# uma-pi1/kge

Hardware: AMD Instinct MI355X
Metric: scored triples/sec (1vsAll, ComplEx d=512) (higher is better)
Workload: dtype bf16; 1 GPU; FB15k-237 shape ComplEx d=512 1vsAll scoring, bf16 tables, f32 scores: the score_sp and score_po blocks of a batch per step (KgeModel.score_sp_po), batches issued in groups of `group` -- one persistent launch per group (kge_score_queries_multi), which also builds the next group's query vectors; group k on HIP stream k % `group_launches_in_flight`; score rows on a 256-byte pitch; num_entities_per_gpu=14541, num_relations=237, dim=512, batch=512, group=8, group_launches_in_flight=1, parallelism=single GPU, queries=split (q_hi + q_lo)

## Files before the change

### kge_amd/csrc/score_pairs_bf16_v8.hip

```cpp
#include "common.hpp"
#include "bf16_queries.hpp"
#include <atomic>
#include <cstdlib>

namespace kge {

constexpr int V8_UT = 32;
constexpr int V8_BAND_CAP = 255;
constexpr int V8_PB = 14;
constexpr unsigned int V8_DROP = 0x80000000u;

struct V8Args {
  Operand TG;
  long long n, m;
  int rgn1;
  int sides;
  int chunks;
  int nbatch;
  long long q_stride;
  long long out_stride;
  long long out2_off, ldo;
  int nunits, su, wpx;
  float* out;
  const u32x4* qf;
  unsigned long long* dbg;
  NextQ nx;
};

#define KGE_V8_DMA(D, VO, P) \
  KGE_STALL(__LINE__ + 7000); \
  asm volatile("s_mov_b32 m0, %0\n\ts_nop 0\n\tglobal_load_lds_dwordx4 %1, %2" : : "s"(D), "v"(VO), "s"(P) : "memory", "m0")

template <int SCORER, int SPLIT, int AUX, int VAR = 0>
__global__ __launch_bounds__(512, 1) void pairs_bf16_v8_kernel(V8Args a) {
  constexpr int HH = 256;
  constexpr int NKB = 2 * HH / 16;
  constexpr int ROWB = 4 * HH;
  constexpr int UNITB = V8_UT * ROWB;
  constexpr int NBUF = 4;
  constexpr int SMEM = NBUF * UNITB;
  constexpr int RW = SPLIT ? 16 : 32;
  constexpr int NST = SPLIT ? 8 : 16;
  constexpr int PF = SPLIT ? 4 : 8;
  static_assert(NKB % PF == 0 && PF <= 8, "look-ahead depth");
  constexpr int FR0 = 12;
  constexpr int VMN_STEADY = (NST > 15 ? 1 : 0) + NST + 4 + V8_PB / 2;
  constexpr int VMN = VMN_STEADY - 2;
  static_assert(VMN <= (NST > 15 ? 9 : 1) + (NKB - FR0 - 14) + 4 + V8_PB / 2, "the chain behind the cold chain");
  __shared__ __attribute__((aligned(16))) unsigned char smem[SMEM];
  if (a.n < 0) smem[threadIdx.x] = 0;

  const int b = blockIdx.x;
  const int x = b & 7, j = b >> 3;
  const int tid = threadIdx.x, lane = tid & 63;
  const int wave = __builtin_amdgcn_readfirstlane(tid >> 6);
  int u_lo = x * a.su;
  int sux = a.nunits - u_lo;
  if (sux > a.su) sux = a.su;
  const int P = a.nbatch * a.sides * a.chunks;
  const int g0 = 0;
  int g1 = 0, pair0 = 0, pstep = a.wpx;
  if (sux > 0) {
    if (P >= a.wpx) {
      pair0 = j;
      g1 = j < P ? ((P - j + a.wpx - 1) / a.wpx) * sux : 0;
    } else {
      const int nsub = a.wpx / P;
      if (j < P * nsub) {
        pair0 = j % P;
        const int sub = j / P;
        const int lo = (int)((long long)sux * sub / nsub), hi = (int)((long long)sux * (sub + 1) / nsub);
        u_lo += lo;
        sux = hi - lo;
        g1 = sux;
      }
    }
  }

  int dbg_i = 0;
  auto stamp = [&]() {
    if (a.dbg != nullptr && tid == 0 && dbg_i < 32) a.dbg[(long long)blockIdx.x * 64 + dbg_i] = __builtin_readcyclecounter();
    ++dbg_i;
  };
  auto stamp_at = [&](int slot) {
    if (a.dbg != nullptr && tid == 0) a.dbg[(long long)blockIdx.x * 64 + slot] = __builtin_readcyclecounter();
  };

  if (g1 > g0) {
    stamp();
    const unsigned char* const tgb = (const unsigned char*)a.TG.base;
    const long long tld2 = a.TG.ld * 2;
    const long long m = a.m;
    const unsigned int lane16 = (unsigned int)lane << 4;
    const int r4 = 4 * wave;
    const unsigned int dx0 = (unsigned int)((r4 & 15) << 4);
    int dq = g0;
    int du = g0 % sux;
    const int ulast = (g1 - 1) % sux;
    auto dma_piece = [&](int un, int ks, auto kc) __attribute__((always_inline)) {
      constexpr int kk = decltype(kc)::value;
      long long r = (long long)(u_lo + un) * V8_UT + r4 + kk;
      if (r >= m) r = m - 1;
      const unsigned char* pk = tgb + r * tld2;
      const unsigned int dk = (unsigned int)((ks & (NBUF - 1)) * UNITB + (r4 + kk) * ROWB);
      const unsigned int vo = lane16 ^ (dx0 + (unsigned int)(kk << 4));
      KGE_V8_DMA(dk, vo, pk);
    };
    auto dma_advance = [&]() __attribute__((always_inline)) {
      ++dq;
      if (++du == sux) du = 0;
    };
    auto fill_unit = [&](int k) __attribute__((always_inline)) {
      const int un = dq < g1 ? du : ulast;
      v4_static_for<0, 4>([&](auto kc) __attribute__((always_inline)) { dma_piece(un, k, kc); });
      dma_advance();
    };

    const int fi = lane & 31, fh = lane >> 5;
    bf16x8 afr[NKB];
    unsigned int bp[8];
#pragma unroll
    for (int t = 0; t < 8; ++t) bp[t] = (unsigned int)(fi * ROWB + (((2 * t + fh) ^ (fi & 15)) << 4));
    bf16x8 bq[PF];
    auto bread = [&](bf16x8& dst, auto kc) __attribute__((always_inline)) {
      constexpr int kb = decltype(kc)::value;
      const unsigned int addr = bp[kb & 7];
      asm volatile("ds_read_b128 %0, %1 offset:%2" : "=v"(dst) : "v"(addr), "i"((kb >> 3) * 256) : "memory");
    };
    const unsigned int ldo4 = (unsigned int)(a.ldo * 4);
    const unsigned int svo = (unsigned int)(((long long)(4 * fh) * a.ldo + fi) * 4);
    __amdgpu_buffer_rsrc_t srs = __builtin_amdgcn_make_buffer_rsrc((void*)a.out, 0, 0, 0x00020000);
    auto store_q = [&](const f32x16& acc, auto qc, unsigned int vo, unsigned int colb) __attribute__((always_inline)) {
      constexpr int q = decltype(qc)::value;
      constexpr int r = SPLIT ? (q & 3) + 8 * (q >> 2) : q;
      constexpr int rowc = SPLIT ? 8 * (r >> 3) + (r & 3) : 8 * (r >> 2) + (r & 3);
      const unsigned int vr = vo + (unsigned int)rowc * ldo4;
      float v = acc[r];
      if constexpr (SPLIT) {
        const float lo = acc[r + 4];
        v = v + lo;
      }
      if constexpr (VAR & 1) {
        asm volatile("" : : "v"(v), "v"(vr));
      } else {
        __builtin_amdgcn_raw_buffer_store_b32(__builtin_bit_cast(unsigned int, v), srs, vr, colb, AUX);
      }
    };
    auto unit_vo = [&](int cu, unsigned int& colb) __attribute__((always_inline)) -> unsigned int {
      const long long col0 = (long long)(u_lo + cu) * V8_UT;
      colb = (unsigned int)(col0 * 4);
      return (col0 + V8_UT <= m || col0 + fi < m) ? svo : V8_DROP;
    };

    f32x16 acc0, acc1;
    auto chain = [&](int ks, f32x16& acc, const f32x16& prev, unsigned int vo, unsigned int colb, auto cold, auto&& frag)
        __attribute__((always_inline)) {
      constexpr bool COLD = decltype(cold)::value;
      const unsigned int bdelta = ((ks + 1) & (NBUF - 1)) ? (unsigned int)UNITB : (unsigned int)(-(NBUF - 1) * UNITB);
      int un = dq < g1 ? du : ulast;
      v4_static_for<0, NKB>([&](auto kc) __attribute__((always_inline)) {
        constexpr int kb = decltype(kc)::value;
        asm volatile("s_waitcnt lgkmcnt(%0)" ::"i"(PF - 1) : "memory");
        if constexpr (kb == V8_PB) {
          asm volatile("s_waitcnt vmcnt(%0)" ::"i"(COLD ? 25 : VMN) : "memory");
          KGE_BARRIER();
        }
        __builtin_amdgcn_sched_barrier(0);
        if constexpr (kb == 0) {
          const f32x16 zero = {0, 0, 0, 0, 0, 0, 0, 0, 0, 0, 0, 0, 0, 0, 0, 0};
          acc = __builtin_amdgcn_mfma_f32_32x32x16_bf16(afr[0], bq[0], zero, 0, 0, 0);
        } else {
          acc = __builtin_amdgcn_mfma_f32_32x32x16_bf16(afr[kb], bq[kb % PF], acc, 0, 0, 0);
        }
        if constexpr (kb + PF == NKB) {
#pragma unroll
          for (int t = 0; t < 8; ++t) asm volatile("v_add_u32 %0, %1, %0" : "+v"(bp[t]) : "s"(bdelta));
        }
        bread(bq[kb % PF], std::integral_constant<int, (kb + PF) % NKB>{});
        if constexpr ((kb & 1) == 0 && kb / 2 < NST) store_q(prev, std::integral_constant<int, kb / 2>{}, vo, colb);
        if constexpr (COLD && kb < NKB - FR0) frag(std::integral_constant<int, FR0 + kb>{});
        if constexpr (COLD && kb < 14 && (kb & 3) == 1) dma_piece(un, ks + 2, std::integral_constant<int, kb / 4>{});
        if constexpr (COLD && kb == 14) {
          dma_advance();
          un = dq < g1 ? du : ulast;
        }
        if constexpr (kb >= 17 && ((kb - 17) & 3) == 0) dma_piece(un, ks + 3, std::integral_constant<int, (kb - 17) / 4>{});
      });
      dma_advance();
      stamp();
    };
    using Cold = std::true_type;
    using Warm = std::false_type;
    auto nofrag = [](auto) {};

    int g = g0, ks = 0;
    int pair = pair0;
    const int cu = 0;
    bool first = true;
    while (g < g1) {
      const int cnt = sux;
      const int per = a.sides * a.chunks;
      const int lb = pair / per, rem = pair - lb * per;
      const int side = rem / a.chunks, ch = rem - side * a.chunks;
      const long long rb = (long long)ch * (8 * RW) + RW * wave;
      long long rows_here = rb < a.n ? (a.n - rb < RW ? a.n - rb : RW) : 0;
      float* const ob = a.out + (long long)lb * a.out_stride + (side ? a.out2_off : 0) + (rows_here > 0 ? rb : 0) * a.ldo;
      srs = __builtin_amdgcn_make_buffer_rsrc((void*)ob, 0, (int)(rows_here * a.ldo * 4), 0x00020000);
      int grp = 2 * ch + (wave >> 2);
      if (grp >= a.rgn1) grp = a.rgn1 - 1;
      grp += side * a.rgn1;
      const unsigned char* const gbase = (const unsigned char*)(a.qf + (long long)lb * a.q_stride + (long long)grp * 4 * NKB * 64);
      unsigned int flo;
      const unsigned char* fb;
      int frange;
      if constexpr (SPLIT) {
        const int part = (fi >> 3) & 1, rr = 16 * (wave & 3) + 8 * (fi >> 4) + (fi & 7);
        flo = (unsigned int)((((2 * part + (rr >> 5)) * NKB) * 64 + (rr & 31) + 32 * fh) * 16);
        fb = gbase;
        frange = 4 * NKB * 1024;
      } else {
        flo = (unsigned int)(lane * 16);
        fb = gbase + (wave & 3) * (NKB * 1024);
        frange = NKB * 1024;
      }
      const __amdgpu_buffer_rsrc_t frs = __builtin_amdgcn_make_buffer_rsrc((void*)fb, 0, frange, 0x00020000);
      auto load_fragments = [&](auto lo, auto hi) __attribute__((always_inline)) {
        v4_static_for<decltype(lo)::value, decltype(hi)::value>([&](auto kc) __attribute__((always_inline)) {
          constexpr int kb = decltype(kc)::value;
          afr[kb] = __builtin_bit_cast(bf16x8, __builtin_amdgcn_raw_buffer_load_b128(frs, flo + kb * 1024, 0, 16 ));
        });
      };
      using C0 = std::integral_constant<int, 0>;
      using CF = std::integral_constant<int, FR0>;
      using C32 = std::integral_constant<int, NKB>;
      unsigned int pvo = V8_DROP, pcolb = 0;
      if (first) {
        fill_unit(0);
        load_fragments(C0{}, CF{});
        asm volatile("s_waitcnt vmcnt(%0)" ::"i"(FR0) : "memory");
        KGE_BARRIER();
        stamp();
        fill_unit(1);
        v4_static_for<0, PF>([&](auto jc) __attribute__((always_inline)) { bread(bq[decltype(jc)::value], jc); });
        first = false;
        chain(ks, acc0, acc1, pvo, pcolb, Cold{}, [&](auto kc) __attribute__((always_inline)) {
          load_fragments(kc, std::integral_constant<int, decltype(kc)::value + 1>{});
        });
      } else {
        load_fragments(C0{}, C32{});
        chain(ks, acc0, acc1, pvo, pcolb, Warm{}, nofrag);
      }
      pvo = unit_vo(cu, pcolb);
      ++ks;
      int i = 1;
      for (; i + 1 < cnt; i += 2) {
        chain(ks, acc1, acc0, pvo, pcolb, Warm{}, nofrag);
        pvo = unit_vo(cu + i, pcolb);
        chain(ks + 1, acc0, acc1, pvo, pcolb, Warm{}, nofrag);
        pvo = unit_vo(cu + i + 1, pcolb);
        ks += 2;
      }
      if (i < cnt) {
        chain(ks, acc1, acc0, pvo, pcolb, Warm{}, nofrag);
        pvo = unit_vo(cu + i, pcolb);
        ++ks;
        v4_static_for<0, NST>([&](auto qc) __attribute__((always_inline)) { store_q(acc1, qc, pvo, pcolb); });
      } else {
        v4_static_for<0, NST>([&](auto qc) __attribute__((always_inline)) { store_q(acc0, qc, pvo, pcolb); });
      }
      g += cnt;
      pair += pstep;
    }
    asm volatile("s_waitcnt lgkmcnt(0)" ::: "memory");
    if constexpr (PF == 8)
      asm volatile("" : : "v"(bq[0]), "v"(bq[1]), "v"(bq[2]), "v"(bq[3]), "v"(bq[4]), "v"(bq[5]), "v"(bq[6]), "v"(bq[7]));
    else
      asm volatile("" : : "v"(bq[0]), "v"(bq[1]), "v"(bq[2]), "v"(bq[3]));
    stamp_at(34);
  }
  if (a.nx.qf != nullptr)
    v4_build_queries<SCORER, HH, SPLIT>(a.nx, (long long)blockIdx.x * 512 + threadIdx.x, (long long)gridDim.x * 512);
}

void v6_set_stamps(unsigned long long* p);
unsigned long long* v6_get_stamps();

int run_pairs_bf16_v8_store256(const Operand& TG, bool split, bool two_sided, long long n, long long m, int nbatch,
                               const void* qf, long long q_stride_bytes, float* out, long long out_stride, long long ldo,
                               long long out2_off, int sc1, int reserve_cus, hipStream_t st);

static int v8_cu_count() {
  static std::atomic<int> cache[64];
  int dev = 0;
  if (hipGetDevice(&dev) != hipSuccess) return 0;
  if (dev >= 0 && dev < 64) {
    const int c = cache[dev].load(std::memory_order_relaxed);
    if (c > 0) return c;
  }
  int v = 0;
  if (hipDeviceGetAttribute(&v, hipDeviceAttributeMultiprocessorCount, dev) != hipSuccess) return 0;
  if (dev >= 0 && dev < 64) cache[dev].store(v, std::memory_order_relaxed);
  return v;
}

static int g_v8_launches[2] = {0, 0};
int v8_launch_count(int which) { return (which == 0 || which == 1) ? __atomic_load_n(&g_v8_launches[which], __ATOMIC_RELAXED) : -1; }

template <int SCORER, int SPLIT>
static int launch_v8(V8Args& a, int sc1, hipStream_t st) {
  int cus = v8_cu_count();
  (void)cus;
  __atomic_fetch_add(&g_v8_launches[0], 1, __ATOMIC_RELAXED);
  const dim3 grid(8 * a.wpx), block(512);
#ifdef KGE_V8_PROBES
  if constexpr (SCORER == KGE_COMPLEX && SPLIT == 1) {
    if (sw(SW_V8_VAR) == 1) {
      hipLaunchKernelGGL((pairs_bf16_v8_kernel<SCORER, SPLIT, 2, 1>), grid, block, 0, st, a);
      return hipGetLastError() == hipSuccess ? KGE_OK : KGE_ERR_LAUNCH;
    }
  }
#endif
  if (sc1 == 1)
    hipLaunchKernelGGL((pairs_bf16_v8_kernel<SCORER, SPLIT, 16>), grid, block, 0, st, a);
  else if (sc1 == 2)
    hipLaunchKernelGGL((pairs_bf16_v8_kernel<SCORER, SPLIT, 2>), grid, block, 0, st, a);
  else if (sc1 == 3)
    hipLaunchKernelGGL((pairs_bf16_v8_kernel<SCORER, SPLIT, 18>), grid, block, 0, st, a);
  else
    hipLaunchKernelGGL((pairs_bf16_v8_kernel<SCORER, SPLIT, 0>), grid, block, 0, st, a);
  return hipGetLastError() == hipSuccess ? KGE_OK : KGE_ERR_LAUNCH;
}

int run_pairs_bf16_v8(int scorer, bool split, const Operand& TG, bool two_sided, int d, long long n, long long m,
                      int nbatch, const void* qf, long long q_stride_bytes, float* out, long long out_stride,
                      long long ldo, long long out2_off, hipStream_t st, unsigned long long* dbg, const NextQ& nx,
                      int reserve_cus) {
  if ((d != 512 && d != 256) || TG.idx.ptr != nullptr || qf == nullptr || nbatch < 1) return KGE_ERR_UNSUPPORTED;
  const long long e = sw(SW_V8);
  if (e == 0) return KGE_ERR_UNSUPPORTED;
  if (nbatch == 1 && e != 1) return KGE_ERR_UNSUPPORTED;
  if (TG.ld * 2 >= (1LL << 28) || ldo >= (1LL << 24)) return KGE_ERR_UNSUPPORTED;
  if ((q_stride_bytes & 15) || ((uintptr_t)qf & 15)) return KGE_ERR_INVALID_ARG;
  const long long rgr = split ? 64 : 128;
  const long long rgn1 = (n + rgr - 1) / rgr;
  const long long pairs = (long long)nbatch * (two_sided ? 2 : 1) * ((rgn1 + 1) / 2);
  const long long nunits = (m + V8_UT - 1) / V8_UT;
  if (rgn1 > (1 << 20) || pairs * nunits >= (1LL << 30)) return KGE_ERR_UNSUPPORTED;
  int cus = v8_cu_count() - reserve_cus;
  if (cus > 256) cus = 256;
  if (cus < 8) cus = 8;
  V8Args a{};
  a.TG = TG;
  a.n = n;
  a.m = m;
  a.rgn1 = (int)rgn1;
  a.sides = two_sided ? 2 : 1;
  a.chunks = (int)((rgn1 + 1) / 2);
  a.nbatch = nbatch;
  a.q_stride = q_stride_bytes / 16;
  a.out_stride = out_stride;
  a.out2_off = out2_off;
  a.ldo = ldo;
  a.nunits = (int)nunits;
  a.su = (int)((nunits + 7) / 8);
  a.wpx = cus / 8;
  a.out = out;
  a.qf = (const u32x4*)qf;
  a.dbg = dbg != nullptr ? dbg : v6_get_stamps();
  a.nx = nx;
  const long long sc1e = sw(SW_V4_STORE_SC1);
  const bool st_aligned = (ldo & 7) == 0 && (out2_off & 7) == 0 && (out_stride & 7) == 0 && ((uintptr_t)out & 31) == 0;
  const double bytes = (double)nbatch * (double)n * (double)m * 4.0 * (two_sided ? 2 : 1);
  const int sc1 = sc1e >= 0 ? (int)sc1e : (!st_aligned ? 0 : (bytes > 160e6 ? 2 : (bytes <= 48e6 ? 1 : 0)));
  if (d == 256) {
    if (nx.qf != nullptr) return KGE_ERR_INVALID_ARG;
    const int pol = sc1e >= 0 ? (int)(sc1e & 3) : (st_aligned && bytes > 1e9 ? 1 : 0);
    const int rc = run_pairs_bf16_v8_store256(TG, split, two_sided, n, m, nbatch, qf, q_stride_bytes, out, out_stride, ldo,
                                              out2_off, pol, reserve_cus, st);
    if (rc == KGE_OK) __atomic_fetch_add(&g_v8_launches[0], 1, __ATOMIC_RELAXED);
    return rc;
  }
#define KGE_V8L(SC) return split ? launch_v8<SC, 1>(a, sc1, st) : launch_v8<SC, 0>(a, sc1, st)
  if (scorer == KGE_COMPLEX) { KGE_V8L(KGE_COMPLEX); }
  if (scorer == KGE_DISTMULT) { KGE_V8L(KGE_DISTMULT); }
#undef KGE_V8L
  return KGE_ERR_UNSUPPORTED;
}


struct V8RankArgs {
  Operand TG;
  long long n, m;
  int rgn1, sides, chunks;
  int nunits, su, wpx;
  const u32x4* qf;
  unsigned long long* dbg;
  CeArgs ce;
};

template <int SCORER, int HH, int SPLIT, int PROBE = 0, int BAND = 0>
__global__ __launch_bounds__(512, 1) void pairs_bf16_v8_rank_kernel(V8RankArgs a) {
  static_assert(!BAND || !SPLIT, "the band launch runs the q_hi chains only");
  constexpr bool DUP = SPLIT && HH == 256;
  constexpr int PARTS = (SPLIT && HH == 128) ? 2 : 1;
  constexpr int FSETS = PARTS;
  constexpr int NT = (HH == 128 && !SPLIT) ? 2 : 1;
  constexpr int NACC = NT * PARTS;
  constexpr int UT = V8_UT * NT;
  constexpr int NKB = 2 * HH / 16;
  constexpr int ROWB = 4 * HH;
  constexpr int SPR = ROWB / 16;
  constexpr int RPP = 64 / SPR;
  constexpr int UNITB = UT * ROWB;
  constexpr int SUBB = V8_UT * ROWB;
  constexpr int NBUF = 4;
  constexpr int SMEM = NBUF * UNITB;
  constexpr int NP = UNITB / 1024 / 8;
  constexpr int RW = DUP ? 16 : 32;
  constexpr int PF = 4;
  constexpr int PB = NKB == 32 ? 14 : 6;
  constexpr bool RAWFAST = HH == 128;
  __shared__ __attribute__((aligned(16))) unsigned char smem[SMEM];
  if (a.n < 0) smem[threadIdx.x] = 0;

  const int b = blockIdx.x;
  const int x = b & 7, j = b >> 3;
  const int tid = threadIdx.x, lane = tid & 63;
  const int wave = __builtin_amdgcn_readfirstlane(tid >> 6);
  int u_lo = x * a.su;
  int sux = a.nunits - u_lo;
  if (sux > a.su) sux = a.su;
  const int P = a.sides * a.chunks;
  const int g0 = 0;
  int g1 = 0, pair0 = 0, pstep = a.wpx;
  if (sux > 0) {
    if (P >= a.wpx) {
      pair0 = j;
      g1 = j < P ? ((P - j + a.wpx - 1) / a.wpx) * sux : 0;
    } else {
      const int nsub = a.wpx / P;
      if (j < P * nsub) {
        pair0 = j % P;
        const int sub = j / P;
        const int lo = (int)((long long)sux * sub / nsub), hi = (int)((long long)sux * (sub + 1) / nsub);
        u_lo += lo;
        sux = hi - lo;
        g1 = sux;
      }
    }
  }
  if (g1 <= g0) return;
  int dbg_i = 0;
  auto stamp = [&]() {
    if (a.dbg != nullptr && tid == 0 && dbg_i < 32) a.dbg[(long long)blockIdx.x * 64 + dbg_i] = __builtin_readcyclecounter();
    ++dbg_i;
  };
  stamp();
  if (a.dbg != nullptr && tid == 0) a.dbg[(long long)blockIdx.x * 64 + 42] = wall_clock64();

  const unsigned char* const tgb = (const unsigned char*)a.TG.base;
  const long long tld2 = a.TG.ld * 2;
  const long long m = a.m;
  const int lr = lane / SPR, slot = lane % SPR;
  const int rp0 = wave * NP * RPP;
  int dq = g0, du = g0 % sux;
  const int ulast = (g1 - 1) % sux;
  auto dma_piece = [&](int un, int ks, auto kc) __attribute__((always_inline)) {
    constexpr int kk = decltype(kc)::value;
    const int ru = rp0 + kk * RPP;
    const long long r0 = (long long)(u_lo + un) * UT + ru;
    const unsigned int dk = (unsigned int)((ks & (NBUF - 1)) * UNITB + ru * ROWB);
    const unsigned int sw = (unsigned int)((slot ^ ((ru + lr) & 15)) << 4);
    const long long rb = r0 < m ? r0 : m - 1;
    const unsigned char* pk = tgb + rb * tld2;
    unsigned int vo = sw;
    if constexpr (RPP > 1) {
      const int left = (int)(m - 1 - rb < RPP - 1 ? m - 1 - rb : RPP - 1);
      vo += (unsigned int)((lr < left ? lr : left) * (int)tld2);
    }
    KGE_V8_DMA(dk, vo, pk);
  };
  auto dma_advance = [&]() __attribute__((always_inline)) {
    ++dq;
    if (++du == sux) du = 0;
  };
#pragma unroll
  for (int k = 0; k < NBUF - 1; ++k) {
    const int un = dq < g1 ? du : ulast;
    v4_static_for<0, NP>([&](auto kc) __attribute__((always_inline)) { dma_piece(un, k, kc); });
    dma_advance();
  }

  const int fi = lane & 31, fh = lane >> 5;
  bf16x8 afr[FSETS][NKB];
  unsigned int bp[8];
#pragma unroll
  for (int t = 0; t < 8; ++t) bp[t] = (unsigned int)(fi * ROWB + (((2 * t + fh) ^ (fi & 15)) << 4));
  bf16x8 bq[NT][PF];
  auto bread = [&](bf16x8& dst, auto kc, auto ac) __attribute__((always_inline)) {
    constexpr int kb = decltype(kc)::value, sub = decltype(ac)::value;
    const unsigned int addr = bp[kb & 7];
    asm volatile("ds_read_b128 %0, %1 offset:%2" : "=v"(dst) : "v"(addr), "i"((kb >> 3) * 256 + sub * SUBB) : "memory");
  };

  const CeArgs& ce = a.ce;
  const bool counts_here = DUP ? ((fi >> 3) & 1) == 0 : true;
  float rk_t = 0.0f, rk_al = 0.0f;
  float rk_hi = 0.0f, rk_lo = 0.0f;
  int bl_cnt = 0;
  u32x4* bl_list = nullptr;
  bool rk_slow = false, rk_noraw = false;
  int rk_g = 0, rk_c = 0, rk_fg[2] = {0, 0}, rk_fc[2] = {0, 0}, rk_fn[2] = {0, 0};
  const unsigned char* rk_base = (const unsigned char*)a.qf;
  unsigned int rk_off = 0;
  int orow_cur = 0;
  int side_cur = 0;
  auto rk_spread = [](unsigned int d) __attribute__((always_inline)) -> unsigned int {
    return (d & 0xfu) | ((d & 0xf0u) << 4) | ((d & 0xf00u) << 8) | ((d & 0xf000u) << 12);
  };
  auto full_score = [&](float v) __attribute__((always_inline)) -> float {
    if constexpr (DUP) {
      const float o = __builtin_bit_cast(
          float, __builtin_amdgcn_update_dpp(0, __builtin_bit_cast(int, v), 0x128 , 0xf, 0xf, false));
      return v + o;
    } else {
      return v;
    }
  };
  auto rank_unit = [&](const f32x16& pv, int cu, int sub, unsigned int w0, unsigned int w1, bool count_g = true)
      __attribute__((always_inline)) -> unsigned int {
    unsigned int g, c;
    if (BAND && rk_slow) {
      g = 0u;
      c = 0x0f0f0f0fu;
    } else if (rk_slow) {
      g = c = 0u;
#pragma unroll
      for (int r = 0; r < 16; ++r) {
        int g0_ = 0, c0_ = 0;
        count_one(full_score(pv[r]), rk_t, ce.rk_atol, ce.rk_rtol, g0_, c0_);
        const unsigned int bit = 1u << (8 * (r >> 2) + (r & 3));
        g |= g0_ ? bit : 0u;
        c |= c0_ ? bit : 0u;
      }
    } else {
      unsigned int ng = 0u, nc = 0u;
#pragma unroll
      for (int r = 15; r >= 0; --r) {
        float xq;
        asm("v_max_f32 %0, 0xff800000, %1" : "=v"(xq) : "v"(full_score(pv[r])));
        const float e = xq - rk_t;
        ng = __builtin_amdgcn_alignbit(ng, __builtin_bit_cast(unsigned int, rk_al - e), 31);
        nc = __builtin_amdgcn_alignbit(nc, __builtin_bit_cast(unsigned int, rk_al - __builtin_fabsf(e)), 31);
      }
      g = rk_spread(ng & 0xffffu);
      c = rk_spread(~nc & 0xffffu);
    }
    const long long c0t = ((long long)(u_lo + cu) * NT + sub) * V8_UT;
    unsigned int mine = counts_here ? (0x0f0f0f0fu << (4 * fh)) : 0u;
    const long long rem = m - c0t;
    if (rem < V8_UT) mine &= rem > 0 ? (1u << rem) - 1u : 0u;
    g = (g << (4 * fh)) & mine;
    c = (c << (4 * fh)) & mine;
    if (!count_g) return c;
    rk_g += __builtin_popcount(g);
    if constexpr (!BAND) rk_c += __builtin_popcount(c);
    const unsigned int ww[2] = {w0 & mine, w1 & mine};
#pragma unroll
    for (int k = 0; k < 2; ++k) {
      if (k < ce.rk_nfilt) {
        rk_fg[k] += __builtin_popcount(g & ww[k]);
        if constexpr (!BAND) rk_fc[k] += __builtin_popcount(c & ww[k]);
        rk_fn[k] += __builtin_popcount(ww[k]);
      }
    }
    return c;
  };
  auto rank_unit_raw = [&](const f32x16& pv) __attribute__((always_inline)) -> int {
    int g = 0, c2 = 0;
#pragma unroll
    for (int r = 0; r < 16; ++r) {
      const float x = full_score(pv[r]);
      g += x > rk_hi ? 1 : 0;
      c2 += x >= rk_lo ? 1 : 0;
    }
    rk_g += g;
    if constexpr (!BAND) rk_c += c2 - g;
    return c2 - g;
  };
  auto rank_flush = [&]() __attribute__((always_inline)) {
    const int G = rk_g + __shfl_xor(rk_g, 32, 64), C = rk_c + __shfl_xor(rk_c, 32, 64);
    const bool wr = counts_here && orow_cur < a.n && fh == 0;
    unsigned long long* rank = ce.rk_rank[side_cur] + orow_cur;
    unsigned long long* ties = ce.rk_ties[side_cur] + orow_cur;
    if (wr && G != 0) atomicAdd(rank, (unsigned long long)G);
    if (wr && C != 0) atomicAdd(ties, (unsigned long long)C);
    const int fc = rk_t == -__builtin_inff() ? 1 : 0;
#pragma unroll
    for (int k = 0; k < 2; ++k) {
      if (k < ce.rk_nfilt) {
        const int FG = rk_fg[k] + __shfl_xor(rk_fg[k], 32, 64), FC = rk_fc[k] + __shfl_xor(rk_fc[k], 32, 64);
        const int FN = rk_fn[k] + __shfl_xor(rk_fn[k], 32, 64);
        const int Gk = G - FG, Ck = C - FC + fc * FN;
        if (wr && Gk != 0) atomicAdd(rank + (k + 1) * ce.rk_ld, (unsigned long long)Gk);
        if (wr && Ck != 0) atomicAdd(ties + (k + 1) * ce.rk_ld, (unsigned long long)Ck);
      }
      rk_fg[k] = rk_fc[k] = rk_fn[k] = 0;
    }
    rk_g = rk_c = 0;
  };
  auto load_words = [&](int cu, u32x2 (&w)[NT]) __attribute__((always_inline)) {
#pragma unroll
    for (int sub = 0; sub < NT; ++sub) {
      const unsigned char* wb = rk_base + (ce.rk_nfilt > 0 ? ((long long)(u_lo + cu) * NT + sub) * ce.rk_bits_us * 4 : 0);
      asm volatile("global_load_dwordx2 %0, %1, %2" : "=v"(w[sub]) : "v"(rk_off), "s"(wb) : "memory");
    }
  };

  auto run = [&](auto half) __attribute__((always_inline)) {
    constexpr int HALF = decltype(half)::value;
    constexpr int PBH = HALF ? 0 : PB;
    constexpr int NPV = (PROBE & 2) ? 0 : NP, WV = (PROBE & 8) ? 0 : NT;
    constexpr int VMB = (NBUF - 3) * (NPV + WV) + WV;
    static_assert(VMB + NP + NT < 64, "vmcnt is a 6-bit counter");
    constexpr int VMF = NPV;
    f32x16 acc[NACC];
    u32x2 wc[NT] = {}, wn[NT] = {};
    auto chain = [&](int ks, int cu, int cu_next) __attribute__((always_inline)) {
      const unsigned int bdelta = ((ks + 1) & (NBUF - 1)) ? (unsigned int)UNITB : (unsigned int)(-(NBUF - 1) * UNITB);
      const int un = dq < g1 ? du : ulast;
      v4_static_for<0, NKB>([&](auto kc) __attribute__((always_inline)) {
        constexpr int kb = decltype(kc)::value;
        asm volatile("s_waitcnt lgkmcnt(%0)" ::"i"((PF - 1) * NT) : "memory");
// ... 596 lines not shown
```

Before: 528.1 billion scored triples/s.

## Store score rows as 16-byte lines via DPP quad transpose in split path

```diff
diff --git a/kge_amd/csrc/score_pairs_bf16_v8.hip b/kge_amd/csrc/score_pairs_bf16_v8.hip
--- a/kge_amd/csrc/score_pairs_bf16_v8.hip
+++ b/kge_amd/csrc/score_pairs_bf16_v8.hip
@@ -31,7 +31,30 @@
   KGE_STALL(__LINE__ + 7000); \
   asm volatile("s_mov_b32 m0, %0\n\ts_nop 0\n\tglobal_load_lds_dwordx4 %1, %2" : : "s"(D), "v"(VO), "s"(P) : "memory", "m0")
 
-template <int SCORER, int SPLIT, int AUX, int VAR = 0>
+constexpr int V8_PIECES = 4;
+constexpr int V8_PIECE_SLOT0 = 17, V8_PIECE_STEP = 4;
+constexpr int V8_GROUP_STEPS = 6;
+constexpr int v8_group_slot(int split, int g) { return split ? 6 * g : (g < 2 ? 6 * g : 15 + 7 * (g - 2)); }
+constexpr int v8_stores(int split, int wide) { return wide ? (split ? 2 : 4) : (split ? 8 : 16); }
+constexpr int v8_store_slot(int split, int wide, int q) { return wide ? v8_group_slot(split, q) + V8_GROUP_STEPS - 1 : 2 * q; }
+constexpr int v8_stores_in(int split, int wide, int lo, int hi) {
+  int c = 0;
+  for (int q = 0; q < v8_stores(split, wide); ++q) c += (v8_store_slot(split, wide, q) >= lo && v8_store_slot(split, wide, q) < hi) ? 1 : 0;
+  return c;
+}
+constexpr bool v8_is_piece_slot(int kb) { return kb >= V8_PIECE_SLOT0 && (kb - V8_PIECE_SLOT0) % V8_PIECE_STEP == 0 && (kb - V8_PIECE_SLOT0) / V8_PIECE_STEP < V8_PIECES; }
+constexpr int V8_LAST_PIECE_SLOT = V8_PIECE_SLOT0 + (V8_PIECES - 1) * V8_PIECE_STEP;
+constexpr bool v8_store_slots_ok(int split, int wide) {
+  for (int q = 0; q < v8_stores(split, wide); ++q) {
+    const int s = v8_store_slot(split, wide, q);
+    if (s < 0 || s >= 32) return false;
+    if (wide && (s == V8_PB || v8_is_piece_slot(s))) return false;
+    if (q > 0 && s <= v8_store_slot(split, wide, q - 1)) return false;
+  }
+  return true;
+}
+
+template <int SCORER, int SPLIT, int AUX, int VAR = 0, int WIDE = 0>
 __global__ __launch_bounds__(512, 1) void pairs_bf16_v8_kernel(V8Args a) {
   constexpr int HH = 256;
   constexpr int NKB = 2 * HH / 16;
@@ -40,13 +63,29 @@
   constexpr int NBUF = 4;
   constexpr int SMEM = NBUF * UNITB;
   constexpr int RW = SPLIT ? 16 : 32;
-  constexpr int NST = SPLIT ? 8 : 16;
+  constexpr int NG = SPLIT ? 2 : 4;
+  constexpr int NST = v8_stores(SPLIT, WIDE);
+  constexpr int NSTD = v8_stores(SPLIT, 0);
+  static_assert(v8_store_slots_ok(SPLIT, WIDE), "store slots");
   constexpr int PF = SPLIT ? 4 : 8;
   static_assert(NKB % PF == 0 && PF <= 8, "look-ahead depth");
   constexpr int FR0 = 12;
-  constexpr int VMN_STEADY = (NST > 15 ? 1 : 0) + NST + 4 + V8_PB / 2;
-  constexpr int VMN = VMN_STEADY - 2;
-  static_assert(VMN <= (NST > 15 ? 9 : 1) + (NKB - FR0 - 14) + 4 + V8_PB / 2, "the chain behind the cold chain");
+  constexpr int ST_LT_PB = v8_stores_in(SPLIT, WIDE, 0, V8_PB);
+  constexpr int ST_GE_PB = NST - ST_LT_PB;
+  constexpr int ST_GT_LASTP = v8_stores_in(SPLIT, WIDE, V8_LAST_PIECE_SLOT + 1, NKB);
+  constexpr int COLD_PIECES_LT_PB = 4;
+  static_assert(V8_PB == 14 && V8_LAST_PIECE_SLOT == 29 && V8_PIECES == 4, "the slots the counts below are written for");
+  constexpr int VMN_STEADY = ST_GT_LASTP + NST + V8_PIECES + ST_LT_PB;
+  constexpr int VMN_COLD = ST_LT_PB + V8_PB + COLD_PIECES_LT_PB;
+  constexpr int VMN_AFTER_COLD = ST_GE_PB + (NKB - FR0 - V8_PB) + V8_PIECES + ST_LT_PB;
+  constexpr int VMN_BOUNDARY = VMN_STEADY + NG + NKB;
+  constexpr int VMN = VMN_STEADY < VMN_AFTER_COLD ? VMN_STEADY : VMN_AFTER_COLD;
+  static_assert(VMN <= VMN_STEADY && VMN <= VMN_AFTER_COLD && VMN <= VMN_BOUNDARY, "the counted wait of the warm chains");
+  static_assert(VMN_COLD == v8_stores_in(SPLIT, WIDE, 0, V8_PB) + 14 + 4 && FR0 + V8_PB <= NKB, "the cold chain");
+  static_assert(WIDE || (VMN_COLD == 25 && VMN_STEADY == (SPLIT ? 19 : 28) && VMN_AFTER_COLD == (SPLIT ? 18 : 26)),
+                "the dword form's counts as they were counted by hand");
+  static_assert(!WIDE || (VMN_COLD == 20 && VMN_STEADY == (SPLIT ? 8 : 10) && VMN_AFTER_COLD == (SPLIT ? 12 : 14)),
+                "the line form's counts");
   __shared__ __attribute__((aligned(16))) unsigned char smem[SMEM];
   if (a.n < 0) smem[threadIdx.x] = 0;
 
@@ -143,13 +182,105 @@
       if constexpr (VAR & 1) {
         asm volatile("" : : "v"(v), "v"(vr));
       } else {
+        if constexpr (WIDE) KGE_STALL(__LINE__ + 7000);
         __builtin_amdgcn_raw_buffer_store_b32(__builtin_bit_cast(unsigned int, v), srs, vr, colb, AUX);
+      }
+    };
+    const unsigned int svo_w = (unsigned int)(((long long)(4 * fh + (lane & 3)) * a.ldo + (fi & ~3)) * 4);
+    unsigned int tw[4] = {0u, 0u, 0u, 0u};
+    const unsigned long long m_odd = __builtin_amdgcn_ballot_w64((lane & 1) != 0), m_up = __builtin_amdgcn_ballot_w64((lane & 2) != 0);
+    unsigned int tl[2] = {0u, 0u};
+#define KGE_V8_CND_DPP(PAD, VCCOP, QP)                                                                              \
+  asm volatile(PAD VCCOP " vcc, %4\n\t"                                                                             \
+               "v_cndmask_b32_dpp %0, %2, %5, vcc quad_perm:" QP " row_mask:0xf bank_mask:0xf\n\t"                   \
+               "v_cndmask_b32_dpp %1, %3, %6, vcc quad_perm:" QP " row_mask:0xf bank_mask:0xf"                        \
+               : "=&v"(d0), "=&v"(d1) : "v"(p0), "v"(p1), "s"(mask), "v"(k0), "v"(k1) : "vcc")
+    auto cnd_dpp = [&](unsigned int& d0, unsigned int& d1, unsigned int p0, unsigned int p1, unsigned int k0, unsigned int k1,
+                       unsigned long long mask, auto inv, auto dist, auto inchain) __attribute__((always_inline)) {
+      constexpr bool INV = decltype(inv)::value, D2 = decltype(dist)::value == 2, PAD = !decltype(inchain)::value;
+      if constexpr (PAD) {
+        if constexpr (INV) { if constexpr (D2) KGE_V8_CND_DPP("s_nop 1\n\t", "s_not_b64", "[2,3,0,1]"); else KGE_V8_CND_DPP("s_nop 1\n\t", "s_not_b64", "[1,0,3,2]"); }
+        else { if constexpr (D2) KGE_V8_CND_DPP("s_nop 1\n\t", "s_mov_b64", "[2,3,0,1]"); else KGE_V8_CND_DPP("s_nop 1\n\t", "s_mov_b64", "[1,0,3,2]"); }
+      } else {
+        if constexpr (INV) { if constexpr (D2) KGE_V8_CND_DPP("", "s_not_b64", "[2,3,0,1]"); else KGE_V8_CND_DPP("", "s_not_b64", "[1,0,3,2]"); }
+        else { if constexpr (D2) KGE_V8_CND_DPP("", "s_mov_b64", "[2,3,0,1]"); else KGE_V8_CND_DPP("", "s_mov_b64", "[1,0,3,2]"); }
+      }
+    };
+#undef KGE_V8_CND_DPP
+    using Dist1 = std::integral_constant<int, 1>;
+    using Dist2 = std::integral_constant<int, 2>;
+    auto store_w = [&](const f32x16& acc, auto gc, auto sc, unsigned int vo, unsigned int colb, auto inchain)
+        __attribute__((always_inline)) {
+      constexpr int g = decltype(gc)::value, s = decltype(sc)::value;
+      static_assert(g < NG && s < V8_GROUP_STEPS, "group step");
+      if constexpr (s == 0) {
+#pragma unroll
+        for (int jj = 0; jj < 4; ++jj) {
+          float v = acc[(SPLIT ? 8 : 4) * g + jj];
+          if constexpr (SPLIT) {
+            const float lo = acc[8 * g + 4 + jj];
+            v = v + lo;
+          }
+          tw[jj] = __builtin_bit_cast(unsigned int, v);
+        }
+      } else if constexpr (s == 1) {
+        cnd_dpp(tl[0], tl[1], tw[1], tw[3], tw[0], tw[2], m_odd, std::true_type{}, Dist1{}, inchain);
+      } else if constexpr (s == 2) {
+        cnd_dpp(tw[1], tw[3], tw[0], tw[2], tw[1], tw[3], m_odd, std::false_type{}, Dist1{}, inchain);
+        tw[0] = tl[0];
+        tw[2] = tl[1];
+      } else if constexpr (s == 3) {
+        cnd_dpp(tl[0], tl[1], tw[2], tw[3], tw[0], tw[1], m_up, std::true_type{}, Dist2{}, inchain);
+      } else if constexpr (s == 4) {
+        cnd_dpp(tw[2], tw[3], tw[0], tw[1], tw[2], tw[3], m_up, std::false_type{}, Dist2{}, inchain);
+        tw[0] = tl[0];
+        tw[1] = tl[1];
+      } else {
+        const unsigned int vr = vo + (unsigned int)(8 * g) * ldo4;
+        if constexpr (VAR & 1) {
+          asm volatile("" : : "v"(tw[0]), "v"(tw[1]), "v"(tw[2]), "v"(tw[3]), "v"(vr));
+        } else {
+          const u32x4 w = {tw[0], tw[1], tw[2], tw[3]};
+          KGE_STALL(__LINE__ + 7000);
+          __builtin_amdgcn_raw_buffer_store_b128(w, srs, vr, colb, AUX);
+          if constexpr (decltype(inchain)::value)
+            asm volatile("" : : "v"(w));
+          else
+            asm volatile("s_nop 7" : : "v"(w));
+        }
+      }
+    };
+    auto store_slot = [&](const f32x16& prev, auto kc, unsigned int vo, unsigned int colb) __attribute__((always_inline)) {
+      constexpr int kb = decltype(kc)::value;
+      if constexpr (WIDE) {
+        v4_static_for<0, NG>([&](auto gc) __attribute__((always_inline)) {
+          constexpr int s = kb - v8_group_slot(SPLIT, decltype(gc)::value);
+          if constexpr (s >= 0 && s < V8_GROUP_STEPS) store_w(prev, gc, std::integral_constant<int, s>{}, vo, colb, std::true_type{});
+        });
+      } else {
+        if constexpr ((kb & 1) == 0 && kb / 2 < NST) store_q(prev, std::integral_constant<int, kb / 2>{}, vo, colb);
       }
     };
     auto unit_vo = [&](int cu, unsigned int& colb) __attribute__((always_inline)) -> unsigned int {
       const long long col0 = (long long)(u_lo + cu) * V8_UT;
       colb = (unsigned int)(col0 * 4);
+      if constexpr (WIDE) return col0 + V8_UT <= m ? svo_w : V8_DROP;
       return (col0 + V8_UT <= m || col0 + fi < m) ? svo : V8_DROP;
+    };
+    auto flush_unit = [&](const f32x16& acc, unsigned int vo, unsigned int colb) __attribute__((always_inline)) {
+      if constexpr (WIDE) {
+        const long long col0 = (long long)(colb >> 2);
+        if (col0 + V8_UT <= m) {
+          v4_static_for<0, NG>([&](auto gc) __attribute__((always_inline)) {
+            v4_static_for<0, V8_GROUP_STEPS>([&](auto sc) __attribute__((always_inline)) { store_w(acc, gc, sc, vo, colb, std::false_type{}); });
+          });
+        } else {
+          const unsigned int dvo = col0 + fi < m ? svo : V8_DROP;
+          v4_static_for<0, NSTD>([&](auto qc) __attribute__((always_inline)) { store_q(acc, qc, dvo, colb); });
+        }
+      } else {
+        v4_static_for<0, NST>([&](auto qc) __attribute__((always_inline)) { store_q(acc, qc, vo, colb); });
+      }
     };
 
     f32x16 acc0, acc1;
@@ -162,7 +293,7 @@
         constexpr int kb = decltype(kc)::value;
         asm volatile("s_waitcnt lgkmcnt(%0)" ::"i"(PF - 1) : "memory");
         if constexpr (kb == V8_PB) {
-          asm volatile("s_waitcnt vmcnt(%0)" ::"i"(COLD ? 25 : VMN) : "memory");
+          asm volatile("s_waitcnt vmcnt(%0)" ::"i"(COLD ? VMN_COLD : VMN) : "memory");
           KGE_BARRIER();
         }
         __builtin_amdgcn_sched_barrier(0);
@@ -177,14 +308,15 @@
           for (int t = 0; t < 8; ++t) asm volatile("v_add_u32 %0, %1, %0" : "+v"(bp[t]) : "s"(bdelta));
         }
         bread(bq[kb % PF], std::integral_constant<int, (kb + PF) % NKB>{});
-        if constexpr ((kb & 1) == 0 && kb / 2 < NST) store_q(prev, std::integral_constant<int, kb / 2>{}, vo, colb);
+        store_slot(prev, kc, vo, colb);
         if constexpr (COLD && kb < NKB - FR0) frag(std::integral_constant<int, FR0 + kb>{});
         if constexpr (COLD && kb < 14 && (kb & 3) == 1) dma_piece(un, ks + 2, std::integral_constant<int, kb / 4>{});
         if constexpr (COLD && kb == 14) {
           dma_advance();
           un = dq < g1 ? du : ulast;
         }
-        if constexpr (kb >= 17 && ((kb - 17) & 3) == 0) dma_piece(un, ks + 3, std::integral_constant<int, (kb - 17) / 4>{});
+        if constexpr (v8_is_piece_slot(kb))
+          dma_piece(un, ks + 3, std::integral_constant<int, (kb - V8_PIECE_SLOT0) / V8_PIECE_STEP>{});
       });
       dma_advance();
       stamp();
@@ -264,9 +396,9 @@
         chain(ks, acc1, acc0, pvo, pcolb, Warm{}, nofrag);
         pvo = unit_vo(cu + i, pcolb);
         ++ks;
-        v4_static_for<0, NST>([&](auto qc) __attribute__((always_inline)) { store_q(acc1, qc, pvo, pcolb); });
+        flush_unit(acc1, pvo, pcolb);
       } else {
-        v4_static_for<0, NST>([&](auto qc) __attribute__((always_inline)) { store_q(acc0, qc, pvo, pcolb); });
+        flush_unit(acc0, pvo, pcolb);
       }
       g += cnt;
       pair += pstep;
@@ -303,32 +435,44 @@
   return v;
 }
 
-static int g_v8_launches[2] = {0, 0};
-int v8_launch_count(int which) { return (which == 0 || which == 1) ? __atomic_load_n(&g_v8_launches[which], __ATOMIC_RELAXED) : -1; }
-
-template <int SCORER, int SPLIT>
-static int launch_v8(V8Args& a, int sc1, hipStream_t st) {
-  int cus = v8_cu_count();
-  (void)cus;
-  __atomic_fetch_add(&g_v8_launches[0], 1, __ATOMIC_RELAXED);
+static int g_v8_launches[3] = {0, 0, 0};
+int v8_launch_count(int which) { return (which >= 0 && which <= 2) ? __atomic_load_n(&g_v8_launches[which], __ATOMIC_RELAXED) : -1; }
+
+constexpr bool V8_WIDE_SINGLE_PASS = false;
+
+template <int SCORER, int SPLIT, int WIDE>
+static int launch_v8w(V8Args& a, int sc1, hipStream_t st) {
   const dim3 grid(8 * a.wpx), block(512);
 #ifdef KGE_V8_PROBES
   if constexpr (SCORER == KGE_COMPLEX && SPLIT == 1) {
     if (sw(SW_V8_VAR) == 1) {
-      hipLaunchKernelGGL((pairs_bf16_v8_kernel<SCORER, SPLIT, 2, 1>), grid, block, 0, st, a);
+      hipLaunchKernelGGL((pairs_bf16_v8_kernel<SCORER, SPLIT, 2, 1, WIDE>), grid, block, 0, st, a);
       return hipGetLastError() == hipSuccess ? KGE_OK : KGE_ERR_LAUNCH;
     }
   }
 #endif
   if (sc1 == 1)
-    hipLaunchKernelGGL((pairs_bf16_v8_kernel<SCORER, SPLIT, 16>), grid, block, 0, st, a);
+    hipLaunchKernelGGL((pairs_bf16_v8_kernel<SCORER, SPLIT, 16, 0, WIDE>), grid, block, 0, st, a);
   else if (sc1 == 2)
-    hipLaunchKernelGGL((pairs_bf16_v8_kernel<SCORER, SPLIT, 2>), grid, block, 0, st, a);
+    hipLaunchKernelGGL((pairs_bf16_v8_kernel<SCORER, SPLIT, 2, 0, WIDE>), grid, block, 0, st, a);
   else if (sc1 == 3)
-    hipLaunchKernelGGL((pairs_bf16_v8_kernel<SCORER, SPLIT, 18>), grid, block, 0, st, a);
+    hipLaunchKernelGGL((pairs_bf16_v8_kernel<SCORER, SPLIT, 18, 0, WIDE>), grid, block, 0, st, a);
   else
-    hipLaunchKernelGGL((pairs_bf16_v8_kernel<SCORER, SPLIT, 0>), grid, block, 0, st, a);
+    hipLaunchKernelGGL((pairs_bf16_v8_kernel<SCORER, SPLIT, 0, 0, WIDE>), grid, block, 0, st, a);
   return hipGetLastError() == hipSuccess ? KGE_OK : KGE_ERR_LAUNCH;
+}
+
+template <int SCORER, int SPLIT>
+static int launch_v8(V8Args& a, int sc1, hipStream_t st) {
+  __atomic_fetch_add(&g_v8_launches[0], 1, __ATOMIC_RELAXED);
+  const bool rows16 = (a.ldo & 3) == 0 && (a.out2_off & 3) == 0 && (a.out_stride & 3) == 0 && ((uintptr_t)a.out & 15) == 0;
+  if constexpr (SPLIT == 1 || V8_WIDE_SINGLE_PASS) {
+    if (rows16) {
+      __atomic_fetch_add(&g_v8_launches[2], 1, __ATOMIC_RELAXED);
+      return launch_v8w<SCORER, SPLIT, 1>(a, sc1, st);
+    }
+  }
+  return launch_v8w<SCORER, SPLIT, 0>(a, sc1, st);
 }
 
 int run_pairs_bf16_v8(int scorer, bool split, const Operand& TG, bool two_sided, int d, long long n, long long m,
```

Result: no change. 525.9 billion scored triples/s (-0.4%).
